# atarashansky/scrna-parameter-estimation

Hardware: NVIDIA B200
Metric: genes tested/sec (ht_1d, num_boot=10k) (higher is better)
Workload: dtype f64

## Files before the change

scrna-parameter-estimation_b200/csrc/gev.cu:

```cuda
#include "common.cuh"
#include <float.h>

namespace mm {

constexpr int kGevThreads = 64;
constexpr int kLadder = 9;
__constant__ int c_tail_n[kLadder] = {300, 270, 240, 210, 180, 150, 120, 90, 60};
__constant__ double c_ks_crit[kLadder] = {0.07783200514647708, 0.08200786390881423, 0.08693932047855427,
                                          0.09288606396320713, 0.100252942300571,   0.1097143944417969,
                                          0.12250018407843426, 0.1411693954054822,  0.1723049003305659};
constexpr double kPenalty = 709.782712893384 * 100.0;

struct GevParams {
    const double* coef_rows;
    const int* flagged;
    const int* extreme;
    int max_extreme;
    int n_flag, B, sort_cap;
    double* asl;
    int* status;
};

__device__ double gev_nnlf(const double* x, int n, double c, double loc, double scale, int lane) {
    if (!isfinite(c) || !(scale > 0.0)) return INFINITY;
    double acc = 0.0;
    int bad = 0;
    const double sup = (c > 0.0) ? 1.0 / fmax(c, DBL_MIN) : ((c < 0.0) ? 1.0 / fmin(c, -DBL_MIN) : 0.0);
    for (int i = lane; i < n; i += 32) {
        double z = (x[i] - loc) / scale;
        bool inside = (c > 0.0) ? (z < sup) : ((c < 0.0) ? (z > sup) : true);
        if (!inside || !(z == z)) { ++bad; continue; }
        double lp;
        if (c != 0.0) {
            double cx = c * z;
            double lex2 = log1p(-cx);
            double lpex2 = lex2 / c;
            lp = (cx == 1.0 || cx == -INFINITY) ? -INFINITY : (-exp(lpex2) + lpex2 - lex2);
        } else {
            lp = -exp(-z) - z;
        }
        if (isfinite(lp)) acc -= lp; else ++bad;
    }
    acc = warp_sum(acc);
    bad = warp_sum_int(bad);
    return acc + (bad > 0 ? bad * kPenalty : 0.0) + (double)n * log(scale);
}

__device__ double gev_logcdf_inner(double z, double c) {
    return (c != 0.0) ? -exp(log1p(-c * z) / c) : -exp(-z);
}
__device__ double gev_cdf(double xv, double c, double loc, double scale) {
    double z = (xv - loc) / scale;
    if (c > 0.0 && z >= 1.0 / c) return 1.0;
    if (c < 0.0 && z <= 1.0 / c) return 0.0;
    return exp(gev_logcdf_inner(z, c));
}
__device__ double gev_sf(double xv, double c, double loc, double scale) {
    double z = (xv - loc) / scale;
    if (c > 0.0 && z >= 1.0 / c) return 0.0;
    if (c < 0.0 && z <= 1.0 / c) return 1.0;
    return -expm1(gev_logcdf_inner(z, c));
}

__device__ void gev_fitstart(const double* x, int n, int lane, double th[3]) {
    double s = 0.0, mn = INFINITY, mx = -INFINITY;
    for (int i = lane; i < n; i += 32) { s += x[i]; mn = fmin(mn, x[i]); mx = fmax(mx, x[i]); }
    s = warp_sum(s);
#pragma unroll
    for (int o = 16; o > 0; o >>= 1) {
        mn = fmin(mn, __shfl_xor_sync(kFull, mn, o));
        mx = fmax(mx, __shfl_xor_sync(kFull, mx, o));
    }
    const double mu = s / n;
    double m2 = 0.0, m3 = 0.0;
    for (int i = lane; i < n; i += 32) { double d = x[i] - mu; m2 += d * d; m3 += d * d * d; }
    m2 = warp_sum(m2) / n;
    m3 = warp_sum(m3) / n;
    const double c = (m3 / pow(m2, 1.5) < 0.0) ? 0.5 : -0.5;
    double loc, scale;
    if (c > 0.0) {
        scale = sqrt(m2 / 0.8584073464102069);
        loc = mu - scale * 0.227546149094484;
        if (!isfinite(loc)) loc = 0.0;
        if (!(isfinite(scale) && scale > 0.0)) scale = 1.0;
        const double b = 2.0;
        if (!(mx < loc + b * scale)) { loc = (mx - b) + 0.1 * (mx - mn); scale = 1.0; }
    } else {
        loc = mu; scale = 1.0;
        const double a = -2.0;
        if (!(loc + a * scale < mn)) { loc = (mn - a) - 0.1 * (mx - mn); scale = 1.0; }
    }
    th[0] = c; th[1] = loc; th[2] = scale;
}

__device__ bool gev_fit(const double* x, int n, int lane, double best[3]) {
    double sim[4][3], fsim[4];
    double x0[3];
    gev_fitstart(x, n, lane, x0);
    for (int k = 0; k < 3; ++k) sim[0][k] = x0[k];
    for (int j = 0; j < 3; ++j) {
        for (int k = 0; k < 3; ++k) sim[j + 1][k] = x0[k];
        sim[j + 1][j] = (x0[j] != 0.0) ? 1.05 * x0[j] : 0.00025;
    }
    int fcalls = 0;
    for (int j = 0; j < 4; ++j) { fsim[j] = gev_nnlf(x, n, sim[j][0], sim[j][1], sim[j][2], lane); ++fcalls; }
    auto sort4 = [&]() {
        for (int i = 1; i < 4; ++i) {
            double f = fsim[i], v0 = sim[i][0], v1 = sim[i][1], v2 = sim[i][2];
            int j = i - 1;
            while (j >= 0 && fsim[j] > f) {
                fsim[j + 1] = fsim[j];
                sim[j + 1][0] = sim[j][0]; sim[j + 1][1] = sim[j][1]; sim[j + 1][2] = sim[j][2];
                --j;
            }
            fsim[j + 1] = f; sim[j + 1][0] = v0; sim[j + 1][1] = v1; sim[j + 1][2] = v2;
        }
    };
    sort4();
    const int maxit = 600, maxfun = 600;
    int it = 0;
    while (fcalls < maxfun && it < maxit) {
        double dx = 0.0, df = 0.0;
        for (int j = 1; j < 4; ++j) {
            for (int k = 0; k < 3; ++k) dx = fmax(dx, fabs(sim[j][k] - sim[0][k]));
            df = fmax(df, fabs(fsim[0] - fsim[j]));
        }
        if (dx <= 1e-4 && df <= 1e-4) break;
        double xbar[3], xr[3];
        for (int k = 0; k < 3; ++k) {
            xbar[k] = (sim[0][k] + sim[1][k] + sim[2][k]) / 3.0;
            xr[k] = 2.0 * xbar[k] - sim[3][k];
        }
        double fxr = gev_nnlf(x, n, xr[0], xr[1], xr[2], lane); ++fcalls;
        bool shrink = false;
        if (fxr < fsim[0]) {
            double xe[3];
            for (int k = 0; k < 3; ++k) xe[k] = 3.0 * xbar[k] - 2.0 * sim[3][k];
            double fxe = gev_nnlf(x, n, xe[0], xe[1], xe[2], lane); ++fcalls;
            if (fxe < fxr) { for (int k = 0; k < 3; ++k) sim[3][k] = xe[k]; fsim[3] = fxe; }
            else { for (int k = 0; k < 3; ++k) sim[3][k] = xr[k]; fsim[3] = fxr; }
        } else if (fxr < fsim[2]) {
            for (int k = 0; k < 3; ++k) sim[3][k] = xr[k];
            fsim[3] = fxr;
        } else if (fxr < fsim[3]) {
            double xc[3];
            for (int k = 0; k < 3; ++k) xc[k] = 1.5 * xbar[k] - 0.5 * sim[3][k];
            double fxc = gev_nnlf(x, n, xc[0], xc[1], xc[2], lane); ++fcalls;
            if (fxc <= fxr) { for (int k = 0; k < 3; ++k) sim[3][k] = xc[k]; fsim[3] = fxc; }
            else shrink = true;
        } else {
            double xcc[3];
            for (int k = 0; k < 3; ++k) xcc[k] = 0.5 * xbar[k] + 0.5 * sim[3][k];
            double fxcc = gev_nnlf(x, n, xcc[0], xcc[1], xcc[2], lane); ++fcalls;
            if (fxcc < fsim[3]) { for (int k = 0; k < 3; ++k) sim[3][k] = xcc[k]; fsim[3] = fxcc; }
            else shrink = true;
        }
        if (shrink) {
            for (int j = 1; j < 4; ++j) {
                for (int k = 0; k < 3; ++k) sim[j][k] = sim[0][k] + 0.5 * (sim[j][k] - sim[0][k]);
                fsim[j] = gev_nnlf(x, n, sim[j][0], sim[j][1], sim[j][2], lane); ++fcalls;
            }
        }
        sort4();
        ++it;
    }
    best[0] = sim[0][0]; best[1] = sim[0][1]; best[2] = sim[0][2];
    return isfinite(best[0]) && isfinite(best[1]) && (best[2] > 0.0);
}

__device__ double gev_ks(const double* x, int n, const double th[3], int lane) {
    double d = 0.0;
    for (int i = lane; i < n; i += 32) {
        double cdf = gev_cdf(x[i], th[0], th[1], th[2]);
        d = fmax(d, fmax((double)(i + 1) / n - cdf, cdf - (double)i / n));
    }
#pragma unroll
    for (int o = 16; o > 0; o >>= 1) d = fmax(d, __shfl_xor_sync(kFull, d, o));
    return d;
}

constexpr int kCand = 1024;

__device__ void sort_cand(double* a, int tid) {
    for (int k = 2; k <= kCand; k <<= 1)
        for (int j = k >> 1; j > 0; j >>= 1) {
            for (int i = tid; i < kCand; i += kGevThreads) {
                int l = i ^ j;
                if (l > i) {
                    double x = a[i], y = a[l];
                    bool up = ((i & k) == 0);
                    if ((x > y) == up) { a[i] = y; a[l] = x; }
                }
            }
            __syncthreads();
        }
}

__global__ void __launch_bounds__(kGevThreads)
gev_tail_kernel(GevParams P) {
    __shared__ double s_lo[kCand];
    __shared__ double s_hi[kCand];
    __shared__ double s_red[2][kGevThreads / 32];
    __shared__ int s_cnt[3];
    __shared__ int s_state[2][kLadder];
    __shared__ double s_val[2][kLadder];
    const int row = P.flagged ? P.flagged[blockIdx.x] : (int)blockIdx.x;
    if (!P.flagged) {
        const int e = P.extreme[row];
        if (e < 0 || e > P.max_extreme || !isfinite(P.asl[row])) {
            if (threadIdx.x == 0) P.status[blockIdx.x] = -1;
            return;
        }
    }
    const double* cr = P.coef_rows + (long long)row * (P.B + 1);
    const int tid = threadIdx.x, lane = tid & 31, warp = tid >> 5;
    const double stat = cr[0], astat = fabs(stat);
    if (tid < 2 * kLadder) { s_state[tid / kLadder][tid % kLadder] = 0; }
    double sum = 0.0, sq = 0.0;
    int cnt = 0;
    for (int i = tid; i < P.B; i += kGevThreads) {
        double d = cr[i + 1] - stat;
        if (isfinite(d)) { sum += d; sq = fma(d, d, sq); ++cnt; }
    }
    sum = warp_sum(sum); sq = warp_sum(sq); cnt = warp_sum_int(cnt);
    if (tid < 3) s_cnt[tid] = 0;
    if (lane == 0) { s_red[0][warp] = sum; s_red[1][warp] = sq; }
    __syncthreads();
    if (lane == 0) atomicAdd(&s_cnt[0], cnt);
    __syncthreads();
    const int n = s_cnt[0];
    double tsum = 0.0, tsq = 0.0;
    for (int w = 0; w < kGevThreads / 32; ++w) { tsum += s_red[0][w]; tsq += s_red[1][w]; }
    if (n < c_tail_n[0]) {
        if (tid == 0) P.status[blockIdx.x] = 0;
        return;
    }
    const double mu = tsum / n;
    double var = tsq / n - mu * mu;
    const double sd = sqrt(var > 0.0 ? var : 0.0);
    double t_lo = mu - 1.5 * sd, t_hi = mu + 1.5 * sd;
    bool ok_lo = false, ok_hi = false;
    for (int it = 0; it < 24 && !(ok_lo && ok_hi); ++it) {
        int c_lo = 0, c_hi = 0;
        for (int i = tid; i < P.B; i += kGevThreads) {
            double d = cr[i + 1] - stat;
            if (isfinite(d)) { c_lo += (d <= t_lo); c_hi += (d >= t_hi); }
        }
        c_lo = warp_sum_int(c_lo); c_hi = warp_sum_int(c_hi);
        __syncthreads();
        if (tid < 3) s_cnt[tid] = 0;
        __syncthreads();
        if (lane == 0) { atomicAdd(&s_cnt[1], c_lo); atomicAdd(&s_cnt[2], c_hi); }
        __syncthreads();
        c_lo = s_cnt[1]; c_hi = s_cnt[2];
        ok_lo = c_lo >= c_tail_n[0] && c_lo <= kCand;
        ok_hi = c_hi >= c_tail_n[0] && c_hi <= kCand;
        const double step = sd * (it < 8 ? 0.2 : (it < 16 ? 0.05 : 0.0125));
        if (!ok_lo) t_lo += (c_lo < c_tail_n[0]) ? step : -0.5 * step;
        if (!ok_hi) t_hi -= (c_hi < c_tail_n[0]) ? step : -0.5 * step;
    }
    if (!(ok_lo && ok_hi)) {
        if (tid == 0) P.status[blockIdx.x] = 0;
        return;
    }
    for (int i = tid; i < kCand; i += kGevThreads) { s_lo[i] = INFINITY; s_hi[i] = -INFINITY; }
    __syncthreads();
    if (tid < 3) s_cnt[tid] = 0;
    __syncthreads();
    for (int i = tid; i < P.B; i += kGevThreads) {
        double d = cr[i + 1] - stat;
        if (!isfinite(d)) continue;
        if (d <= t_lo) s_lo[atomicAdd(&s_cnt[1], 1)] = d;
        if (d >= t_hi) s_hi[atomicAdd(&s_cnt[2], 1)] = d;
    }
    __syncthreads();
    sort_cand(s_lo, tid);
    sort_cand(s_hi, tid);
    {
        const int side = warp;
        for (int li = 0; li < kLadder; ++li) {
            const int ne = c_tail_n[li];
            const double* x = side == 0 ? s_lo : s_hi + (kCand - ne);
            double th[3];
            int state;
            double val = 0.0;
            if (!gev_fit(x, ne, lane, th)) state = 3;
            else {
                double d = gev_ks(x, ne, th, lane);
                if (d < c_ks_crit[li]) {
                    state = 1;
                    double pr = side == 0 ? gev_cdf(-astat, th[0], th[1], th[2]) : gev_sf(astat, th[0], th[1], th[2]);
                    val = ((double)ne / (double)n) * pr;
                } else state = 2;
            }
            if (lane == 0) { s_state[side][li] = state; s_val[side][li] = val; }
            if (state != 2) break;
        }
    }
    __syncthreads();
    if (tid == 0) {
        double total = 0.0;
        bool ok = true;
        for (int side = 0; side < 2 && ok; ++side) {
            bool found = false;
            for (int li = 0; li < kLadder; ++li) {
                int s = s_state[side][li];
                if (s == 1) { total += s_val[side][li]; found = true; break; }
                if (s == 3 || s == 0) break;
            }
            ok = found;
        }
        if (ok && isfinite(total)) { P.asl[row] = total; P.status[blockIdx.x] = 1; }
        else P.status[blockIdx.x] = 0;
    }
}

}

using namespace mm;

MM_EXPORT int mm_gev_tail_asl(int device, void* stream, const double* coef_rows, const int32_t* flagged,
                              int32_t n_flag, int32_t num_boot, double* asl, int32_t* status,
                              const int32_t* extreme, int32_t max_extreme) {
    if (int s = enter(device)) return s;
    MM_REQUIRE(n_flag >= 0 && num_boot > 0, "n_flag/num_boot");
    if (n_flag == 0) return 0;
    MM_REQUIRE(coef_rows && (flagged || extreme) && asl && status, "null pointer");
    GevParams P;
    P.coef_rows = coef_rows; P.flagged = flagged; P.n_flag = n_flag; P.B = num_boot; P.sort_cap = 0;
    P.asl = asl; P.status = status; P.extreme = extreme; P.max_extreme = max_extreme;
    gev_tail_kernel<<<n_flag, kGevThreads, 0, (cudaStream_t)stream>>>(P);
    return check_launch("mm_gev_tail_asl");
}
```

scrna-parameter-estimation_b200/csrc/regress.cu:

```cuda
#include "common.cuh"

namespace mm {

constexpr int kRegThreads = 256;
constexpr int kMaxT = 4;
constexpr int kRegCmax = 1024;

struct FillParams {
    const double* raw_mean;
    const double* raw_rv;
    const unsigned char* seg_ok;
    const double* true_mean;
    const double* true_rv;
    const int* src_mean;
    const int* src_rv;
    const long long* gene_id;
    int R;
    int B;
    unsigned long long seed;
    double* boot_mean;
    double* boot_var;
    unsigned char* seg_good;
    int* n_valid;
    const int* n_invalid;
};

__device__ __forceinline__ double pick_valid(const double* row, int B, int n_valid, Philox& rng) {
    for (int it = 0; it < 256; ++it) {
        int j = (int)(rng.uniform() * (float)B);
        if (j >= B) j = B - 1;
        double v = row[j];
        if (v > 0.0) return v;
    }
    int want = (int)(rng.uniform() * (float)n_valid);
    if (want >= n_valid) want = n_valid - 1;
    for (int j = 0; j < B; ++j) {
        double v = row[j];
        if (v > 0.0 && want-- == 0) return v;
    }
    return nan("");
}

__global__ void __launch_bounds__(kRegThreads)
fill_log_kernel(FillParams P) {
    __shared__ int s_cnt[2];
    const long long seg = blockIdx.x;
    const int B = P.B;
    double* om = P.boot_mean + seg * (long long)(B + 1);
    double* ov = P.boot_var + seg * (long long)(B + 1);
    const double* rm = P.raw_mean + seg * (long long)B;
    const double* rr = P.raw_rv + seg * (long long)B;
    if (threadIdx.x < 2) s_cnt[threadIdx.x] = 0;
    __syncthreads();
    bool ok = P.seg_ok[seg] != 0;
    if (ok) {
        int cm = 0, cr = 0;
        for (int b = threadIdx.x; b < B; b += kRegThreads) {
            cm += (rm[b] > 0.0);
            cr += (rr[b] > 0.0);
        }
        cm = warp_sum_int(cm);
        cr = warp_sum_int(cr);
        if ((threadIdx.x & 31) == 0) { atomicAdd(&s_cnt[0], cm); atomicAdd(&s_cnt[1], cr); }
    }
    __syncthreads();
    const int nvm = s_cnt[0], nvr = s_cnt[1];
    ok = ok && nvm > 0 && nvr > 0;
    if (threadIdx.x == 0) {
        P.seg_good[seg] = ok ? 1 : 0;
        P.n_valid[2 * seg] = nvm;
        P.n_valid[2 * seg + 1] = nvr;
    }
    if (!ok) {
        for (int b = threadIdx.x; b <= B; b += kRegThreads) { om[b] = nan(""); ov[b] = nan(""); }
        return;
    }
    if (threadIdx.x == 0) { om[0] = log(P.true_mean[seg]); ov[0] = log(P.true_rv[seg]); }
    const long long sid = P.gene_id ? P.gene_id[seg / P.R] * P.R + (seg % P.R) : seg;
    for (int b = threadIdx.x; b < B; b += kRegThreads) {
        double m = rm[b], v = rr[b];
        if (!(m > 0.0)) {
            if (P.src_mean) m = rm[P.src_mean[seg * (long long)B + b]];
            else {
                Philox rng;
                rng.init(P.seed, (uint32_t)b, (uint32_t)sid, (uint32_t)(sid >> 32), 0xF111u);
                m = pick_valid(rm, B, nvm, rng);
            }
        }
        if (!(v > 0.0)) {
            if (P.src_rv) v = rr[P.src_rv[seg * (long long)B + b]];
            else {
                Philox rng;
                rng.init(P.seed, (uint32_t)b, (uint32_t)sid, (uint32_t)(sid >> 32), 0xF112u);
                v = pick_valid(rr, B, nvr, rng);
            }
        }
        om[b + 1] = log(m);
        ov[b + 1] = log(v);
    }
}

constexpr int kFillMaskWords = 2048;

__device__ __forceinline__ double pick_valid_masked(const double* row, const unsigned* mask, int B, int n_valid, Philox& rng) {
    for (int it = 0; it < 256; ++it) {
        int j = (int)(rng.uniform() * (float)B);
        if (j >= B) j = B - 1;
        if (!((mask[j >> 5] >> (j & 31)) & 1u)) return row[j];
    }
    int want = (int)(rng.uniform() * (float)n_valid);
    if (want >= n_valid) want = n_valid - 1;
    for (int j = 0; j < B; ++j)
        if (!((mask[j >> 5] >> (j & 31)) & 1u) && want-- == 0) return row[j];
    return nan("");
}

__global__ void __launch_bounds__(kRegThreads)
fill_rows_kernel(FillParams P) {
    __shared__ unsigned s_mask[2][kFillMaskWords];
    const long long seg = blockIdx.x;
    const int B = P.B;
    double* om = P.boot_mean + seg * (long long)(B + 1);
    double* ov = P.boot_var + seg * (long long)(B + 1);
    const int im = P.n_invalid[2 * seg], iv = P.n_invalid[2 * seg + 1];
    const int nvm = B - im, nvr = B - iv;
    const bool ok = P.seg_ok[seg] != 0 && nvm > 0 && nvr > 0;
    if (threadIdx.x == 0) {
        P.seg_good[seg] = ok ? 1 : 0;
        P.n_valid[2 * seg] = nvm;
        P.n_valid[2 * seg + 1] = nvr;
    }
    if (!ok) {
        for (int b = threadIdx.x; b <= B; b += kRegThreads) { om[b] = nan(""); ov[b] = nan(""); }
        return;
    }
    if (threadIdx.x == 0) { om[0] = log(P.true_mean[seg]); ov[0] = log(P.true_rv[seg]); }
    if (im == 0 && iv == 0) return;
    const int words = (B + 31) >> 5;
    for (int i = threadIdx.x; i < words; i += kRegThreads) { s_mask[0][i] = 0u; s_mask[1][i] = 0u; }
    __syncthreads();
    for (int b = threadIdx.x; b < B; b += kRegThreads) {
        if (isnan(om[b + 1])) atomicOr(&s_mask[0][b >> 5], 1u << (b & 31));
        if (isnan(ov[b + 1])) atomicOr(&s_mask[1][b >> 5], 1u << (b & 31));
    }
    __syncthreads();
    const long long sid = P.gene_id ? P.gene_id[seg / P.R] * P.R + (seg % P.R) : seg;
    for (int b = threadIdx.x; b < B; b += kRegThreads) {
        if ((s_mask[0][b >> 5] >> (b & 31)) & 1u) {
            Philox rng;
            rng.init(P.seed, (uint32_t)b, (uint32_t)sid, (uint32_t)(sid >> 32), 0xF111u);
            om[b + 1] = pick_valid_masked(om + 1, s_mask[0], B, nvm, rng);
        }
        if ((s_mask[1][b >> 5] >> (b & 31)) & 1u) {
            Philox rng;
            rng.init(P.seed, (uint32_t)b, (uint32_t)sid, (uint32_t)(sid >> 32), 0xF112u);
            ov[b + 1] = pick_valid_masked(ov + 1, s_mask[1], B, nvr, rng);
        }
    }
}

struct WlsParams {
    const double* covariate;
    const double* treatment;
    const double* weights;
    const unsigned char* masks;
    int R, Pc, T, n_mask;
    int T_full;
    const int* col_idx;
    int one_sample;
    int* one_flag;
    double* scratch;
    double* cmat;
    double* znorm2;
};

__device__ double block_sum(double v, double* sred) {
    v = warp_sum(v);
    __syncthreads();
    if ((threadIdx.x & 31) == 0) sred[threadIdx.x >> 5] = v;
    __syncthreads();
    double tot = 0.0;
    for (int w = 0; w < kRegThreads / 32; ++w) tot += sred[w];
    return tot;
}

__global__ void __launch_bounds__(kRegThreads)
wls_functional_kernel(WlsParams P) {
    __shared__ double sred[kRegThreads / 32];
    const int k = blockIdx.x;
    const int R = P.R, Pc = P.Pc, T = P.T, K = Pc + T, TF = P.T_full;
    const unsigned char* mask = P.masks + (long long)k * R;
    double* Z = P.scratch + (long long)k * R * K;
    double* C = P.cmat + (long long)k * T * R;
    const int* cols = P.col_idx ? P.col_idx + (long long)k * T : nullptr;
    const int tid = threadIdx.x;
    auto tcol = [&](int t) { return cols ? cols[t] : t; };

    double wl = 0.0, not_one = 0.0;
    for (int r = tid; r < R; r += kRegThreads) {
        if (!mask[r]) continue;
        wl += P.weights[r];
        for (int t = 0; t < T; ++t) not_one += (P.treatment[(long long)r * TF + tcol(t)] != 1.0) ? 1.0 : 0.0;
    }
    const double wsum = block_sum(wl, sred);
    const bool one_sample = P.one_sample != 0 || block_sum(not_one, sred) == 0.0;
    if (P.one_flag && tid == 0) P.one_flag[k] = one_sample ? 1 : 0;

    if (one_sample) {
        for (int i = tid; i < T * R; i += kRegThreads) {
            int r = i % R;
            C[i] = mask[r] ? P.weights[r] / wsum : 0.0;
        }
        return;
    }
    for (int c = 0; c < K; ++c) {
        double s = 0.0;
        for (int r = tid; r < R; r += kRegThreads) {
            double v = c < Pc ? P.covariate[(long long)r * Pc + c] : P.treatment[(long long)r * TF + tcol(c - Pc)];
            s += mask[r] ? P.weights[r] * v : 0.0;
        }
        double mu = block_sum(s, sred) / wsum;
        for (int r = tid; r < R; r += kRegThreads) {
            double v = c < Pc ? P.covariate[(long long)r * Pc + c] : P.treatment[(long long)r * TF + tcol(c - Pc)];
            Z[(long long)r * K + c] = mask[r] ? v - mu : 0.0;
        }
    }
    __syncthreads();
    for (int c = 0; c < Pc; ++c) {
        double s = 0.0, s0 = 0.0;
        for (int r = tid; r < R; r += kRegThreads) {
            double z = Z[(long long)r * K + c];
            s += P.weights[r] * z * z;
            double v0 = P.covariate[(long long)r * Pc + c];
            s0 += mask[r] ? P.weights[r] * v0 * v0 : 0.0;
        }
        double nrm2 = block_sum(s, sred);
        double ref2 = block_sum(s0, sred);
        const bool dropped = !(nrm2 > 1e-20 * (ref2 > 0.0 ? ref2 : 1.0));
        if (P.znorm2 && tid == 0) P.znorm2[(long long)k * Pc + c] = dropped ? 0.0 : nrm2;
        if (dropped) continue;
        for (int c2 = c + 1; c2 < K; ++c2) {
            double d = 0.0;
            for (int r = tid; r < R; r += kRegThreads)
                d += P.weights[r] * Z[(long long)r * K + c] * Z[(long long)r * K + c2];
            double proj = block_sum(d, sred) / nrm2;
            for (int r = tid; r < R; r += kRegThreads)
                Z[(long long)r * K + c2] -= proj * Z[(long long)r * K + c];
            __syncthreads();
        }
    }
    for (int t = 0; t < T; ++t) {
        double s = 0.0, s0 = 0.0;
        for (int r = tid; r < R; r += kRegThreads) {
            double a = Z[(long long)r * K + Pc + t];
            s += P.weights[r] * a * a;
            double v0 = P.treatment[(long long)r * TF + tcol(t)];
            s0 += mask[r] ? P.weights[r] * v0 * v0 : 0.0;
        }
        double ss = block_sum(s, sred);
        double ref2 = block_sum(s0, sred);
        if (!(ss > 1e-20 * (ref2 > 0.0 ? ref2 : 1.0))) ss = nan("");
        for (int r = tid; r < R; r += kRegThreads)
            C[(long long)t * R + r] = mask[r] ? P.weights[r] * Z[(long long)r * K + Pc + t] / ss : 0.0;
    }
}

struct RegParams {
    const double* boot[2];
    int n_stat;
    const unsigned char* seg_good;
    const int* mask_id;
    const int* gene_list;
    const double* cmat;
    int R, T, B;
    int approx;
    double* coef_ws;
    double* out_coef;
    double* out_se;
    double* out_asl;
    int* out_extreme;
    int* out_nnull;
    int n_split;
    double* split_ws;
};

__device__ __forceinline__ void regress_finish(const RegParams& P, long long o, double stat, double a, double b2, int h,
                                               int l, double vmin, double vmax, int n) {
    double mu = a / n, var = b2 / n - mu * mu;
    if (var < 0) var = 0;
    double sd = sqrt(var);
    double asl;
    int extreme = -1;
    if (!(vmin < vmax)) {
        asl = nan("");
    } else if (P.approx) {
        double astat = fabs(stat), k = 1.0 / (sd * 1.4142135623730951);
        asl = 0.5 * erfc((astat - mu) * k) + 0.5 * erfc((astat + mu) * k);
    } else {
        extreme = h + l;
        asl = (double)(extreme + 1) / (double)(n + 1);
    }
    P.out_coef[o] = stat;
    P.out_se[o] = (n > 0) ? sd : nan("");
    P.out_asl[o] = asl;
    P.out_extreme[o] = extreme;
    P.out_nnull[o] = n;
}

template <int TT>
__global__ void __launch_bounds__(kRegThreads)
regress_asl_kernel(RegParams P) {
    __shared__ double s_stat[2][TT];
    __shared__ double s_red[kRegThreads / 32][2 * TT][2];
    __shared__ int s_cnt[kRegThreads / 32][2 * TT][2];
    __shared__ double s_mm[kRegThreads / 32][2 * TT][2];
    __shared__ int s_nvalid[kRegThreads / 32];
    const int gi = blockIdx.x;
    const int g = P.gene_list ? P.gene_list[gi] : gi;
    const int R = P.R, T = P.T, B1 = P.B + 1, NS = P.n_stat;
    const unsigned char* good = P.seg_good + (long long)g * R;
    const double* C = P.cmat + (long long)P.mask_id[gi] * T * R;
    const int tid = threadIdx.x, lane = tid & 31, warp = tid >> 5;
    __shared__ double s_Cbuf[kRegCmax];
    __shared__ unsigned char s_good[kRegCmax];
    const double* s_C = C;
    if (T * R <= kRegCmax) {
        for (int i = tid; i < T * R; i += kRegThreads) s_Cbuf[i] = C[i];
        for (int i = tid; i < R; i += kRegThreads) s_good[i] = good[i];
        s_C = s_Cbuf;
        good = s_good;
        __syncthreads();
    }

    int n_good = 0;
    for (int r = 0; r < R; ++r) n_good += good[r];
    const long long obase = (long long)gi * NS * T;
    if (n_good == 0) {
        for (int i = tid; i < NS * T && blockIdx.y == 0; i += kRegThreads) {
            P.out_coef[obase + i] = nan(""); P.out_se[obase + i] = nan(""); P.out_asl[obase + i] = nan("");
            P.out_extreme[obase + i] = -1; P.out_nnull[obase + i] = 0;
        }
        return;
    }

    for (int t0 = 0; t0 < T; t0 += TT) {
        const int tn = min(TT, T - t0);
        if (tid < NS * tn) {
            int s = tid / tn, t = tid % tn;
            const double* bt = P.boot[s] + (long long)g * R * B1;
            double acc = 0.0;
            for (int r = 0; r < R; ++r)
                if (good[r]) acc = fma(C[(long long)(t0 + t) * R + r], bt[(long long)r * B1], acc);
            s_stat[s][t] = acc;
        }
        __syncthreads();

        double sum[2][TT], sq[2][TT], mn[2][TT], mx[2][TT];
        int hi[2][TT], lo[2][TT];
#pragma unroll
        for (int s = 0; s < 2; ++s)
#pragma unroll
            for (int t = 0; t < TT; ++t) {
                sum[s][t] = 0; sq[s][t] = 0; hi[s][t] = 0; lo[s][t] = 0;
                mn[s][t] = INFINITY; mx[s][t] = -INFINITY;
            }
        int nvalid = 0;
        const int per = (B1 + P.n_split - 1) / P.n_split;
        const int b_lo = blockIdx.y * per, b_hi = min(B1, b_lo + per);
        for (int b = b_lo + tid; b < b_hi; b += kRegThreads) {
            double acc[2][TT];
#pragma unroll
            for (int s = 0; s < 2; ++s)
#pragma unroll
                for (int t = 0; t < TT; ++t) acc[s][t] = 0.0;
            bool finite = true;
            for (int r0 = 0; r0 < R; r0 += 4) {
                double v[4][2];
#pragma unroll
                for (int j = 0; j < 4; ++j) {
                    const int r = r0 + j;
                    const bool use = r < R && good[r];
#pragma unroll
                    for (int s = 0; s < 2; ++s)
                        v[j][s] = (use && s < NS) ? __ldg(P.boot[s] + ((long long)g * R + r) * B1 + b) : 0.0;
                }
#pragma unroll
                for (int j = 0; j < 4; ++j) {
                    const int r = r0 + j;
                    if (r < R && good[r]) {
#pragma unroll
                        for (int s = 0; s < 2; ++s) {
                            finite = finite && isfinite(v[j][s]);
#pragma unroll
                            for (int t = 0; t < TT; ++t)
                                if (t < tn) acc[s][t] = fma(s_C[(t0 + t) * R + r], v[j][s], acc[s][t]);
                        }
                    }
                }
            }
#pragma unroll
            for (int s = 0; s < 2; ++s) {
                if (s < NS) {
#pragma unroll
                    for (int t = 0; t < TT; ++t) {
                        if (t < tn) {
                            double c = finite ? acc[s][t] : nan("");
                            if (P.coef_ws)
                                P.coef_ws[(((long long)gi * NS + s) * T + t0 + t) * B1 + b] = c;
                            if (finite) {
                                mn[s][t] = fmin(mn[s][t], c);
                                mx[s][t] = fmax(mx[s][t], c);
                                if (b > 0) {
                                    double st = s_stat[s][t];
                                    double d = c - st, a = fabs(st);
                                    sum[s][t] += d;
                                    sq[s][t] = fma(d, d, sq[s][t]);
                                    hi[s][t] += (d > a);
                                    lo[s][t] += (d < -a);
                                }
                            }
                        }
                    }
                }
            }
            if (finite && b > 0) ++nvalid;
        }
        nvalid = warp_sum_int(nvalid);
        if (lane == 0) s_nvalid[warp] = nvalid;
#pragma unroll
        for (int s = 0; s < 2; ++s)
#pragma unroll
            for (int t = 0; t < TT; ++t) {
                if (s < NS && t < tn) {
                    double a = warp_sum(sum[s][t]), b2 = warp_sum(sq[s][t]);
                    int h = warp_sum_int(hi[s][t]), l = warp_sum_int(lo[s][t]);
                    double vmin = mn[s][t], vmax = mx[s][t];
#pragma unroll
                    for (int o = 16; o > 0; o >>= 1) {
                        vmin = fmin(vmin, __shfl_xor_sync(kFull, vmin, o));
                        vmax = fmax(vmax, __shfl_xor_sync(kFull, vmax, o));
                    }
                    if (lane == 0) {
                        s_red[warp][s * TT + t][0] = a; s_red[warp][s * TT + t][1] = b2;
                        s_cnt[warp][s * TT + t][0] = h; s_cnt[warp][s * TT + t][1] = l;
                        s_mm[warp][s * TT + t][0] = vmin; s_mm[warp][s * TT + t][1] = vmax;
                    }
                }
            }
        __syncthreads();
        if (tid < NS * tn) {
            int s = tid / tn, t = tid % tn, j = s * TT + t;
            double a = 0, b2 = 0, vmin = INFINITY, vmax = -INFINITY;
            int h = 0, l = 0, n = 0;
            for (int w = 0; w < kRegThreads / 32; ++w) {
                a += s_red[w][j][0]; b2 += s_red[w][j][1];
                h += s_cnt[w][j][0]; l += s_cnt[w][j][1];
                vmin = fmin(vmin, s_mm[w][j][0]); vmax = fmax(vmax, s_mm[w][j][1]);
                n += s_nvalid[w];
            }
            const double stat = s_stat[s][t];
            const long long o = obase + (long long)s * T + t0 + t;
            if (P.n_split > 1) {
                double* w = P.split_ws + ((((long long)gi * P.n_split + blockIdx.y) * NS + s) * T + t0 + t) * 8;
                w[0] = a; w[1] = b2; w[2] = (double)h; w[3] = (double)l; w[4] = vmin; w[5] = vmax; w[6] = (double)n; w[7] = stat;
            } else {
                regress_finish(P, o, stat, a, b2, h, l, vmin, vmax, n);
            }
        }
        __syncthreads();
    }
}

struct ResampParams {
    double* boot[2];
    int n_stat;
    const unsigned char* seg_good;
    const int* mask_id;
    const int* gene_list;
    const double* zmat;
    const double* znorm2;
    const double* weights;
    int R, Pc, T, B;
    int approx;
    unsigned long long seed;
    const long long* gene_id;
    const int* rep_assign;
    const int* iter_assign;
    double* coef_ws;
    double* out_coef; double* out_se; double* out_asl;
    int* out_extreme; int* out_nnull;
    int* bad_flag;
};

__global__ void __launch_bounds__(kRegThreads)
regress_resampled_kernel(ResampParams P) {
    extern __shared__ int s_good[];
    __shared__ double sred[kRegThreads / 32];
    __shared__ int s_ngood;
    const int gi = blockIdx.x, tid = threadIdx.x;
    const int g = P.gene_list ? P.gene_list[gi] : gi;
    const int R = P.R, Pc = P.Pc, T = P.T, B = P.B, B1 = B + 1, K = Pc + T, NS = P.n_stat;
    const unsigned char* good = P.seg_good + (long long)g * R;
    const double* Z = P.zmat + (long long)P.mask_id[gi] * R * K;
    const double* zn = P.znorm2 + (long long)P.mask_id[gi] * Pc;
    if (tid == 0) {
        int n = 0;
        for (int r = 0; r < R; ++r) if (good[r]) s_good[n++] = r;
        s_ngood = n;
    }
    __syncthreads();
    const int ng = s_ngood;
    const long long obase = (long long)gi * NS * T;
    if (ng == 0) {
        for (int i = tid; i < NS * T; i += kRegThreads) {
            P.out_coef[obase + i] = nan(""); P.out_se[obase + i] = nan(""); P.out_asl[obase + i] = nan("");
            P.out_extreme[obase + i] = -1; P.out_nnull[obase + i] = 0;
        }
        return;
    }
    double wsum = 0.0;
    for (int i = 0; i < ng; ++i) wsum += P.weights[s_good[i]];
    for (int s = 0; s < NS; ++s) {
        double* bt = P.boot[s] + (long long)g * R * B1;
        for (int b = tid; b < B1; b += kRegThreads) {
            double mu = 0.0;
            bool finite = true;
            for (int i = 0; i < ng; ++i) {
                int r = s_good[i];
                double y = bt[(long long)r * B1 + b];
                finite = finite && isfinite(y);
                mu += P.weights[r] * y;
            }
            if (!finite) *P.bad_flag = 1;
            mu /= wsum;
            for (int i = 0; i < ng; ++i) { int r = s_good[i]; bt[(long long)r * B1 + b] -= mu; }
            for (int c = 0; c < Pc; ++c) {
                if (!(zn[c] > 0.0)) continue;
                double d = 0.0;
                for (int i = 0; i < ng; ++i) {
                    int r = s_good[i];
                    d += P.weights[r] * Z[(long long)r * K + c] * bt[(long long)r * B1 + b];
                }
                d /= zn[c];
                for (int i = 0; i < ng; ++i) { int r = s_good[i]; bt[(long long)r * B1 + b] -= d * Z[(long long)r * K + c]; }
            }
        }
    }
    __syncthreads();
    const long long sid_base = (P.gene_id ? P.gene_id[g] : (long long)g) * R;
    auto pick = [&](int i, int j, int& r, int& bi) {
        int ra;
        if (j == 0) { ra = i; bi = 0; }
        else if (P.rep_assign) {
            ra = P.rep_assign[((long long)g * R + i) * B + j];
            bi = P.iter_assign[((long long)g * R + i) * B + j];
        } else {
            Philox rng;
            long long sid = sid_base + i;
            rng.init(P.seed, (uint32_t)j, (uint32_t)sid, (uint32_t)(sid >> 32), 0x4E5Au);
            uint4 r4 = rng.block();
            ra = (int)(((unsigned long long)r4.x * (unsigned)ng) >> 32);
            bi = 1 + (int)(((unsigned long long)r4.y * (unsigned)B) >> 32);
        }
        r = s_good[ra];
    };
    auto slope = [&](const double* bt, int t, int j) {
        double sw = 0, swa = 0, swy = 0, amin = INFINITY, amax = -INFINITY;
        for (int i = 0; i < ng; ++i) {
            int r, bi;
            pick(i, j, r, bi);
            double w = P.weights[r], a = Z[(long long)r * K + Pc + t], y = bt[(long long)r * B1 + bi];
            amin = fmin(amin, a); amax = fmax(amax, a);
            sw = __dadd_rn(sw, w);
            swa = __dadd_rn(swa, __dmul_rn(a, w));
            swy = __dadd_rn(swy, __dmul_rn(y, w));
        }
        if (!(amin < amax)) return nan("");
        const double ma = swa / sw, my = swy / sw;
        double ss = 0, num = 0;
        for (int i = 0; i < ng; ++i) {
            int r, bi;
            pick(i, j, r, bi);
            double w = P.weights[r], a = Z[(long long)r * K + Pc + t], y = bt[(long long)r * B1 + bi];
            double ac = __dadd_rn(a, -ma);
            ss = __dadd_rn(ss, __dmul_rn(__dmul_rn(ac, ac), w));
            num = __dadd_rn(num, __dmul_rn(__dmul_rn(ac, w), __dadd_rn(y, -my)));
        }
        return num / sw / (ss / sw);
    };
    for (int s = 0; s < NS; ++s) {
        const double* bt = P.boot[s] + (long long)g * R * B1;
        for (int t = 0; t < T; ++t) {
            const double stat = slope(bt, t, 0);
            const double astat = fabs(stat);
            double sum = 0, sq = 0, vmin = INFINITY, vmax = -INFINITY;
            int hi = 0, lo = 0, cnt = 0;
            for (int j = tid; j < B; j += kRegThreads) {
                double c = (j == 0) ? stat : slope(bt, t, j);
                if (P.coef_ws) P.coef_ws[(((long long)gi * NS + s) * T + t) * B + j] = c;
                if (!isfinite(c)) continue;
                vmin = fmin(vmin, c); vmax = fmax(vmax, c);
                if (j > 0) {
                    double d = c - stat;
                    sum += d; sq = fma(d, d, sq); hi += (d > astat); lo += (d < -astat); ++cnt;
                }
            }
            sum = block_sum(sum, sred);
            sq = block_sum(sq, sred);
            int ext = (int)(block_sum((double)(hi + lo), sred) + 0.5);
            const int n_fin = (int)(block_sum((double)cnt, sred) + 0.5);
#pragma unroll
            for (int o = 16; o > 0; o >>= 1) {
                vmin = fmin(vmin, __shfl_xor_sync(kFull, vmin, o));
                vmax = fmax(vmax, __shfl_xor_sync(kFull, vmax, o));
            }
            __shared__ double s_mn[kRegThreads / 32], s_mx[kRegThreads / 32];
            if ((tid & 31) == 0) { s_mn[tid >> 5] = vmin; s_mx[tid >> 5] = vmax; }
            __syncthreads();
            if (tid == 0) {
                for (int w = 1; w < kRegThreads / 32; ++w) { vmin = fmin(vmin, s_mn[w]); vmax = fmax(vmax, s_mx[w]); }
                const int n = n_fin;
                double mu = sum / n, var = sq / n - mu * mu;
                if (var < 0) var = 0;
                double sd = sqrt(var), asl;
                int extreme = -1;
                if (!(vmin < vmax)) asl = nan("");
                else if (P.approx) {
                    double k2 = 1.0 / (sd * 1.4142135623730951);
                    asl = 0.5 * erfc((astat - mu) * k2) + 0.5 * erfc((astat + mu) * k2);
                } else { extreme = ext; asl = (double)(ext + 1) / (double)(n + 1); }
                const long long o = obase + (long long)s * T + t;
                P.out_coef[o] = stat; P.out_se[o] = sd; P.out_asl[o] = asl;
                P.out_extreme[o] = extreme; P.out_nnull[o] = n;
            }
            __syncthreads();
        }
    }
}

constexpr int kRsCov = 24;

__device__ __forceinline__ int build_good_list(const unsigned char* good, int R, int* s_good, int* s_n) {
    if (threadIdx.x < 32) {
        const int lane = threadIdx.x;
        int base = 0;
        for (int r0 = 0; r0 < R; r0 += 32) {
            const int r = r0 + lane;
            const bool ok = r < R && good[r];
            const unsigned m = __ballot_sync(kFull, ok);
            if (ok) s_good[base + __popc(m & ((1u << lane) - 1u))] = r;
            base += __popc(m);
        }
        if (lane == 0) *s_n = base;
    }
    __syncthreads();
    return *s_n;
}

constexpr int kRsRows = 32;
constexpr int kRsBatch = 8;

__global__ void __launch_bounds__(kRegThreads, 2)
resample_residualise_kernel(ResampParams P) {
    extern __shared__ int s_good[];
    __shared__ double sred[kRegThreads / 32];
    __shared__ int s_ngood;
    __shared__ __align__(16) double s_z[kRsRows][kRsCov];
    __shared__ double s_w[kRsRows];
    __shared__ int s_r[kRsRows];
    const int gi = blockIdx.x, tid = threadIdx.x;
    const int g = P.gene_list ? P.gene_list[gi] : gi;
    const int R = P.R, Pc = P.Pc, B1 = P.B + 1, K = Pc + P.T;
    const int ng = build_good_list(P.seg_good + (long long)g * R, R, s_good, &s_ngood);
    if (ng == 0) return;
    const double* __restrict__ Z = P.zmat + (long long)P.mask_id[gi] * R * K;
    const double* __restrict__ zn = P.znorm2 + (long long)P.mask_id[gi] * Pc;
    const double* __restrict__ wts = P.weights;
    double wl = 0.0;
    for (int i = tid; i < ng; i += kRegThreads) wl += wts[s_good[i]];
    const double wsum = block_sum(wl, sred);
    const int b = blockIdx.y * kRegThreads + tid;
    const bool active = b < B1;
    auto stage = [&](int i0, int c0, int nc, bool weighted) {
        __syncthreads();
        for (int idx = tid; idx < kRsRows * kRsCov; idx += kRegThreads) {
            const int row = idx / kRsCov, k = idx % kRsCov, i = i0 + row;
            double v = 0.0;
            if (i < ng && k < nc) {
                const int r = s_good[i];
                v = Z[(long long)r * K + c0 + k];
                if (weighted) v *= wts[r];
            }
            s_z[row][k] = v;
        }
        if (tid < kRsRows) {
            const int i = i0 + tid;
            s_r[tid] = s_good[i < ng ? i : ng - 1];
            s_w[tid] = i < ng ? wts[s_r[tid]] : 0.0;
        }
        __syncthreads();
    };
    for (int s = 0; s < P.n_stat; ++s) {
        double* __restrict__ col = P.boot[s] + (long long)g * R * B1 + (active ? b : 0);
        for (int c0 = 0; c0 == 0 || c0 < Pc; c0 += kRsCov) {
            const int nc = min(kRsCov, Pc - c0);
            double acc[kRsCov], mu = 0.0;
#pragma unroll
            for (int k = 0; k < kRsCov; ++k) acc[k] = 0.0;
            bool finite = true;
            for (int i0 = 0; i0 < ng; i0 += kRsRows) {
                stage(i0, c0, nc, true);
                if (!active) continue;
#pragma unroll 1
                for (int u0 = 0; u0 < kRsRows; u0 += kRsBatch) {
                    double y[kRsBatch];
#pragma unroll
                    for (int u = 0; u < kRsBatch; ++u) y[u] = col[(long long)s_r[u0 + u] * B1];
#pragma unroll
                    for (int u = 0; u < kRsBatch; ++u) {
                        finite = finite && (isfinite(y[u]) || s_w[u0 + u] == 0.0);
                        const double yy = s_w[u0 + u] == 0.0 ? 0.0 : y[u];
                        mu = fma(s_w[u0 + u], yy, mu);
                        const double2* zr = reinterpret_cast<const double2*>(s_z[u0 + u]);
#pragma unroll
                        for (int k = 0; k < kRsCov / 2; ++k) {
                            const double2 z2 = zr[k];
                            acc[2 * k] = fma(z2.x, yy, acc[2 * k]);
                            acc[2 * k + 1] = fma(z2.y, yy, acc[2 * k + 1]);
// ... 348 lines not shown
```

Baseline: 44280.

## Widen GEV tail fits to multi-warp sides and unroll regression over columns

The GEV tail kernel grows from one warp per tail side to four warps per side. Each side uses its own named barrier and double-buffered shared term arrays, so the per-point log-likelihood and KS work is spread over 128 threads, and both candidate arrays are sorted in a single bitonic pass. The regression kernel handles two bootstrap columns per thread for TT==1 and widens the row group to 8, which adds independent loads in flight. The cost is more barriers for each Nelder-Mead function evaluation, more shared memory and more registers.

```diff
diff --git a/scrna-parameter-estimation_b200/csrc/gev.cu b/scrna-parameter-estimation_b200/csrc/gev.cu
--- a/scrna-parameter-estimation_b200/csrc/gev.cu
+++ b/scrna-parameter-estimation_b200/csrc/gev.cu
@@ -3,13 +3,18 @@
 
 namespace mm {
 
-constexpr int kGevThreads = 64;
+constexpr int kSideWarps = 4;
+constexpr int kSideThreads = 32 * kSideWarps;
+constexpr int kGevThreads = 2 * kSideThreads;
+constexpr int kMomThreads = 64;
 constexpr int kLadder = 9;
 __constant__ int c_tail_n[kLadder] = {300, 270, 240, 210, 180, 150, 120, 90, 60};
 __constant__ double c_ks_crit[kLadder] = {0.07783200514647708, 0.08200786390881423, 0.08693932047855427,
                                           0.09288606396320713, 0.100252942300571,   0.1097143944417969,
                                           0.12250018407843426, 0.1411693954054822,  0.1723049003305659};
 constexpr double kPenalty = 709.782712893384 * 100.0;
+constexpr int kTailMax = 300;
+constexpr int kPts = (kTailMax + kSideThreads - 1) / kSideThreads;
 
 struct GevParams {
     const double* coef_rows;
@@ -21,24 +26,48 @@
     int* status;
 };
 
-__device__ double gev_nnlf(const double* x, int n, double c, double loc, double scale, int lane) {
+__device__ __forceinline__ void side_sync(int side) {
+    if (side == 0) asm volatile("bar.sync 1, %0;" ::"n"(kSideThreads) : "memory");
+    else asm volatile("bar.sync 2, %0;" ::"n"(kSideThreads) : "memory");
+}
+
+struct SideCtx {
+    int side, st, lane;
+    double* buf;
+    int phase;
+};
+
+__device__ double gev_nnlf(const double* x, int n, double c, double loc, double scale, SideCtx& S) {
     if (!isfinite(c) || !(scale > 0.0)) return INFINITY;
-    double acc = 0.0;
-    int bad = 0;
+    double* lpv = S.buf + S.phase * kTailMax;
+    S.phase ^= 1;
     const double sup = (c > 0.0) ? 1.0 / fmax(c, DBL_MIN) : ((c < 0.0) ? 1.0 / fmin(c, -DBL_MIN) : 0.0);
-    for (int i = lane; i < n; i += 32) {
-        double z = (x[i] - loc) / scale;
-        bool inside = (c > 0.0) ? (z < sup) : ((c < 0.0) ? (z > sup) : true);
-        if (!inside || !(z == z)) { ++bad; continue; }
-        double lp;
-        if (c != 0.0) {
+    if (c != 0.0) {
+#pragma unroll
+        for (int k = 0; k < kPts; ++k) {
+            const int i = S.st + k * kSideThreads;
+            double z = (x[min(i, n - 1)] - loc) / scale;
+            bool inside = (c > 0.0) ? (z < sup) : (z > sup);
             double cx = c * z;
             double lex2 = log1p(-cx);
             double lpex2 = lex2 / c;
-            lp = (cx == 1.0 || cx == -INFINITY) ? -INFINITY : (-exp(lpex2) + lpex2 - lex2);
-        } else {
-            lp = -exp(-z) - z;
-        }
+            double lp = (cx == 1.0 || cx == -INFINITY) ? -INFINITY : (-exp(lpex2) + lpex2 - lex2);
+            if (i < n) lpv[i] = (inside && z == z) ? lp : nan("");
+        }
+    } else {
+#pragma unroll
+        for (int k = 0; k < kPts; ++k) {
+            const int i = S.st + k * kSideThreads;
+            double z = (x[min(i, n - 1)] - loc) / scale;
+            double lp = -exp(-z) - z;
+            if (i < n) lpv[i] = (z == z) ? lp : nan("");
+        }
+    }
+    side_sync(S.side);
+    double acc = 0.0;
+    int bad = 0;
+    for (int i = S.lane; i < n; i += 32) {
+        double lp = lpv[i];
         if (isfinite(lp)) acc -= lp; else ++bad;
     }
     acc = warp_sum(acc);
@@ -93,17 +122,17 @@
     th[0] = c; th[1] = loc; th[2] = scale;
 }
 
-__device__ bool gev_fit(const double* x, int n, int lane, double best[3]) {
+__device__ bool gev_fit(const double* x, int n, SideCtx& S, double best[3]) {
     double sim[4][3], fsim[4];
     double x0[3];
-    gev_fitstart(x, n, lane, x0);
+    gev_fitstart(x, n, S.lane, x0);
     for (int k = 0; k < 3; ++k) sim[0][k] = x0[k];
     for (int j = 0; j < 3; ++j) {
         for (int k = 0; k < 3; ++k) sim[j + 1][k] = x0[k];
         sim[j + 1][j] = (x0[j] != 0.0) ? 1.05 * x0[j] : 0.00025;
     }
     int fcalls = 0;
-    for (int j = 0; j < 4; ++j) { fsim[j] = gev_nnlf(x, n, sim[j][0], sim[j][1], sim[j][2], lane); ++fcalls; }
+    for (int j = 0; j < 4; ++j) { fsim[j] = gev_nnlf(x, n, sim[j][0], sim[j][1], sim[j][2], S); ++fcalls; }
     auto sort4 = [&]() {
         for (int i = 1; i < 4; ++i) {
             double f = fsim[i], v0 = sim[i][0], v1 = sim[i][1], v2 = sim[i][2];
@@ -131,12 +160,12 @@
             xbar[k] = (sim[0][k] + sim[1][k] + sim[2][k]) / 3.0;
             xr[k] = 2.0 * xbar[k] - sim[3][k];
         }
-        double fxr = gev_nnlf(x, n, xr[0], xr[1], xr[2], lane); ++fcalls;
+        double fxr = gev_nnlf(x, n, xr[0], xr[1], xr[2], S); ++fcalls;
         bool shrink = false;
         if (fxr < fsim[0]) {
             double xe[3];
             for (int k = 0; k < 3; ++k) xe[k] = 3.0 * xbar[k] - 2.0 * sim[3][k];
-            double fxe = gev_nnlf(x, n, xe[0], xe[1], xe[2], lane); ++fcalls;
+            double fxe = gev_nnlf(x, n, xe[0], xe[1], xe[2], S); ++fcalls;
             if (fxe < fxr) { for (int k = 0; k < 3; ++k) sim[3][k] = xe[k]; fsim[3] = fxe; }
             else { for (int k = 0; k < 3; ++k) sim[3][k] = xr[k]; fsim[3] = fxr; }
         } else if (fxr < fsim[2]) {
@@ -145,20 +174,20 @@
         } else if (fxr < fsim[3]) {
             double xc[3];
             for (int k = 0; k < 3; ++k) xc[k] = 1.5 * xbar[k] - 0.5 * sim[3][k];
-            double fxc = gev_nnlf(x, n, xc[0], xc[1], xc[2], lane); ++fcalls;
+            double fxc = gev_nnlf(x, n, xc[0], xc[1], xc[2], S); ++fcalls;
             if (fxc <= fxr) { for (int k = 0; k < 3; ++k) sim[3][k] = xc[k]; fsim[3] = fxc; }
             else shrink = true;
         } else {
             double xcc[3];
             for (int k = 0; k < 3; ++k) xcc[k] = 0.5 * xbar[k] + 0.5 * sim[3][k];
-            double fxcc = gev_nnlf(x, n, xcc[0], xcc[1], xcc[2], lane); ++fcalls;
+            double fxcc = gev_nnlf(x, n, xcc[0], xcc[1], xcc[2], S); ++fcalls;
             if (fxcc < fsim[3]) { for (int k = 0; k < 3; ++k) sim[3][k] = xcc[k]; fsim[3] = fxcc; }
             else shrink = true;
         }
         if (shrink) {
             for (int j = 1; j < 4; ++j) {
                 for (int k = 0; k < 3; ++k) sim[j][k] = sim[0][k] + 0.5 * (sim[j][k] - sim[0][k]);
-                fsim[j] = gev_nnlf(x, n, sim[j][0], sim[j][1], sim[j][2], lane); ++fcalls;
+                fsim[j] = gev_nnlf(x, n, sim[j][0], sim[j][1], sim[j][2], S); ++fcalls;
             }
         }
         sort4();
@@ -168,14 +197,18 @@
     return isfinite(best[0]) && isfinite(best[1]) && (best[2] > 0.0);
 }
 
-__device__ double gev_ks(const double* x, int n, const double th[3], int lane) {
+__device__ double gev_ks(const double* x, int n, const double th[3], SideCtx& S, double* red) {
     double d = 0.0;
-    for (int i = lane; i < n; i += 32) {
+    for (int i = S.st; i < n; i += kSideThreads) {
         double cdf = gev_cdf(x[i], th[0], th[1], th[2]);
         d = fmax(d, fmax((double)(i + 1) / n - cdf, cdf - (double)i / n));
     }
 #pragma unroll
     for (int o = 16; o > 0; o >>= 1) d = fmax(d, __shfl_xor_sync(kFull, d, o));
+    if (S.lane == 0) red[S.st >> 5] = d;
+    side_sync(S.side);
+    for (int w = 0; w < kSideWarps; ++w) d = fmax(d, red[w]);
+    side_sync(S.side);
     return d;
 }
 
@@ -184,22 +217,23 @@
 __device__ void sort_cand(double* a, int tid) {
     for (int k = 2; k <= kCand; k <<= 1)
         for (int j = k >> 1; j > 0; j >>= 1) {
-            for (int i = tid; i < kCand; i += kGevThreads) {
-                int l = i ^ j;
+            for (int e = tid; e < 2 * kCand; e += kGevThreads) {
+                const int i = e & (kCand - 1), l = i ^ j;
                 if (l > i) {
-                    double x = a[i], y = a[l];
+                    double* b = a + (e & kCand);
+                    double x = b[i], y = b[l];
                     bool up = ((i & k) == 0);
-                    if ((x > y) == up) { a[i] = y; a[l] = x; }
+                    if ((x > y) == up) { b[i] = y; b[l] = x; }
                 }
             }
             __syncthreads();
         }
 }
 
-__global__ void __launch_bounds__(kGevThreads)
+__global__ void __launch_bounds__(kGevThreads, 2)
 gev_tail_kernel(GevParams P) {
-    __shared__ double s_lo[kCand];
-    __shared__ double s_hi[kCand];
+    __shared__ double s_cand[2][kCand];
+    __shared__ double s_terms[2][2][kTailMax];
     __shared__ double s_red[2][kGevThreads / 32];
     __shared__ int s_cnt[3];
     __shared__ int s_state[2][kLadder];
@@ -216,21 +250,23 @@
     const int tid = threadIdx.x, lane = tid & 31, warp = tid >> 5;
     const double stat = cr[0], astat = fabs(stat);
     if (tid < 2 * kLadder) { s_state[tid / kLadder][tid % kLadder] = 0; }
+    if (tid < 3) s_cnt[tid] = 0;
     double sum = 0.0, sq = 0.0;
     int cnt = 0;
-    for (int i = tid; i < P.B; i += kGevThreads) {
-        double d = cr[i + 1] - stat;
-        if (isfinite(d)) { sum += d; sq = fma(d, d, sq); ++cnt; }
-    }
-    sum = warp_sum(sum); sq = warp_sum(sq); cnt = warp_sum_int(cnt);
-    if (tid < 3) s_cnt[tid] = 0;
-    if (lane == 0) { s_red[0][warp] = sum; s_red[1][warp] = sq; }
-    __syncthreads();
-    if (lane == 0) atomicAdd(&s_cnt[0], cnt);
+    if (tid < kMomThreads) {
+        for (int i = tid; i < P.B; i += kMomThreads) {
+            double d = cr[i + 1] - stat;
+            if (isfinite(d)) { sum += d; sq = fma(d, d, sq); ++cnt; }
+        }
+        sum = warp_sum(sum); sq = warp_sum(sq); cnt = warp_sum_int(cnt);
+        if (lane == 0) { s_red[0][warp] = sum; s_red[1][warp] = sq; }
+    }
+    __syncthreads();
+    if (tid < kMomThreads && lane == 0) atomicAdd(&s_cnt[0], cnt);
     __syncthreads();
     const int n = s_cnt[0];
     double tsum = 0.0, tsq = 0.0;
-    for (int w = 0; w < kGevThreads / 32; ++w) { tsum += s_red[0][w]; tsq += s_red[1][w]; }
+    for (int w = 0; w < kMomThreads / 32; ++w) { tsum += s_red[0][w]; tsq += s_red[1][w]; }
     if (n < c_tail_n[0]) {
         if (tid == 0) P.status[blockIdx.x] = 0;
         return;
@@ -263,37 +299,38 @@
         if (tid == 0) P.status[blockIdx.x] = 0;
         return;
     }
-    for (int i = tid; i < kCand; i += kGevThreads) { s_lo[i] = INFINITY; s_hi[i] = -INFINITY; }
+    for (int i = tid; i < kCand; i += kGevThreads) { s_cand[0][i] = INFINITY; s_cand[1][i] = -INFINITY; }
     __syncthreads();
     if (tid < 3) s_cnt[tid] = 0;
     __syncthreads();
     for (int i = tid; i < P.B; i += kGevThreads) {
         double d = cr[i + 1] - stat;
         if (!isfinite(d)) continue;
-        if (d <= t_lo) s_lo[atomicAdd(&s_cnt[1], 1)] = d;
-        if (d >= t_hi) s_hi[atomicAdd(&s_cnt[2], 1)] = d;
-    }
-    __syncthreads();
-    sort_cand(s_lo, tid);
-    sort_cand(s_hi, tid);
+        if (d <= t_lo) s_cand[0][atomicAdd(&s_cnt[1], 1)] = d;
+        if (d >= t_hi) s_cand[1][atomicAdd(&s_cnt[2], 1)] = d;
+    }
+    __syncthreads();
+    sort_cand(&s_cand[0][0], tid);
     {
-        const int side = warp;
+        SideCtx S;
+        S.side = tid / kSideThreads; S.st = tid % kSideThreads; S.lane = lane;
+        S.buf = &s_terms[S.side][0][0]; S.phase = 0;
         for (int li = 0; li < kLadder; ++li) {
             const int ne = c_tail_n[li];
-            const double* x = side == 0 ? s_lo : s_hi + (kCand - ne);
+            const double* x = S.side == 0 ? s_cand[0] : s_cand[1] + (kCand - ne);
             double th[3];
             int state;
             double val = 0.0;
-            if (!gev_fit(x, ne, lane, th)) state = 3;
+            if (!gev_fit(x, ne, S, th)) state = 3;
             else {
-                double d = gev_ks(x, ne, th, lane);
+                double d = gev_ks(x, ne, th, S, &s_red[S.side][0]);
                 if (d < c_ks_crit[li]) {
                     state = 1;
-                    double pr = side == 0 ? gev_cdf(-astat, th[0], th[1], th[2]) : gev_sf(astat, th[0], th[1], th[2]);
+                    double pr = S.side == 0 ? gev_cdf(-astat, th[0], th[1], th[2]) : gev_sf(astat, th[0], th[1], th[2]);
                     val = ((double)ne / (double)n) * pr;
                 } else state = 2;
             }
-            if (lane == 0) { s_state[side][li] = state; s_val[side][li] = val; }
+            if (S.st == 0) { s_state[S.side][li] = state; s_val[S.side][li] = val; }
             if (state != 2) break;
         }
     }
diff --git a/scrna-parameter-estimation_b200/csrc/regress.cu b/scrna-parameter-estimation_b200/csrc/regress.cu
--- a/scrna-parameter-estimation_b200/csrc/regress.cu
+++ b/scrna-parameter-estimation_b200/csrc/regress.cu
@@ -310,6 +310,7 @@
 template <int TT>
 __global__ void __launch_bounds__(kRegThreads)
 regress_asl_kernel(RegParams P) {
+    constexpr int kCols = TT == 1 ? 2 : 1, kGroups = TT == 4 ? 4 : 8;
     __shared__ double s_stat[2][TT];
     __shared__ double s_red[kRegThreads / 32][2 * TT][2];
     __shared__ int s_cnt[kRegThreads / 32][2 * TT][2];
@@ -367,63 +368,78 @@
         int nvalid = 0;
         const int per = (B1 + P.n_split - 1) / P.n_split;
         const int b_lo = blockIdx.y * per, b_hi = min(B1, b_lo + per);
-        for (int b = b_lo + tid; b < b_hi; b += kRegThreads) {
-            double acc[2][TT];
-#pragma unroll
-            for (int s = 0; s < 2; ++s)
-#pragma unroll
-                for (int t = 0; t < TT; ++t) acc[s][t] = 0.0;
-            bool finite = true;
-            for (int r0 = 0; r0 < R; r0 += 4) {
-                double v[4][2];
-#pragma unroll
-                for (int j = 0; j < 4; ++j) {
+        for (int b0 = b_lo + tid; b0 < b_hi; b0 += kCols * kRegThreads) {
+            double acc[kCols][2][TT];
+            bool finite[kCols];
+#pragma unroll
+            for (int c = 0; c < kCols; ++c) {
+                finite[c] = true;
+#pragma unroll
+                for (int s = 0; s < 2; ++s)
+#pragma unroll
+                    for (int t = 0; t < TT; ++t) acc[c][s][t] = 0.0;
+            }
+            for (int r0 = 0; r0 < R; r0 += kGroups) {
+                double v[kGroups][kCols][2];
+#pragma unroll
+                for (int j = 0; j < kGroups; ++j) {
                     const int r = r0 + j;
                     const bool use = r < R && good[r];
 #pragma unroll
-                    for (int s = 0; s < 2; ++s)
-                        v[j][s] = (use && s < NS) ? __ldg(P.boot[s] + ((long long)g * R + r) * B1 + b) : 0.0;
-                }
-#pragma unroll
-                for (int j = 0; j < 4; ++j) {
+                    for (int s = 0; s < 2; ++s) {
+                        const double* row = P.boot[s] + ((long long)g * R + r) * B1 + b0;
+#pragma unroll
+                        for (int c = 0; c < kCols; ++c)
+                            v[j][c][s] = (use && s < NS && b0 + c * kRegThreads < b_hi) ? __ldg(row + c * kRegThreads) : 0.0;
+                    }
+                }
+#pragma unroll
+                for (int j = 0; j < kGroups; ++j) {
                     const int r = r0 + j;
                     if (r < R && good[r]) {
 #pragma unroll
-                        for (int s = 0; s < 2; ++s) {
-                            finite = finite && isfinite(v[j][s]);
-#pragma unroll
-                            for (int t = 0; t < TT; ++t)
-                                if (t < tn) acc[s][t] = fma(s_C[(t0 + t) * R + r], v[j][s], acc[s][t]);
-                        }
+                        for (int c = 0; c < kCols; ++c)
+#pragma unroll
+                            for (int s = 0; s < 2; ++s) {
+                                finite[c] = finite[c] && isfinite(v[j][c][s]);
+#pragma unroll
+                                for (int t = 0; t < TT; ++t)
+                                    if (t < tn) acc[c][s][t] = fma(s_C[(t0 + t) * R + r], v[j][c][s], acc[c][s][t]);
+                            }
                     }
                 }
             }
 #pragma unroll
-            for (int s = 0; s < 2; ++s) {
-                if (s < NS) {
-#pragma unroll
-                    for (int t = 0; t < TT; ++t) {
-                        if (t < tn) {
-                            double c = finite ? acc[s][t] : nan("");
-                            if (P.coef_ws)
-                                P.coef_ws[(((long long)gi * NS + s) * T + t0 + t) * B1 + b] = c;
-                            if (finite) {
-                                mn[s][t] = fmin(mn[s][t], c);
-                                mx[s][t] = fmax(mx[s][t], c);
-                                if (b > 0) {
-                                    double st = s_stat[s][t];
-                                    double d = c - st, a = fabs(st);
-                                    sum[s][t] += d;
-                                    sq[s][t] = fma(d, d, sq[s][t]);
-                                    hi[s][t] += (d > a);
-                                    lo[s][t] += (d < -a);
+            for (int c = 0; c < kCols; ++c) {
+                const int b = b0 + c * kRegThreads;
+                if (b >= b_hi) break;
+#pragma unroll
+                for (int s = 0; s < 2; ++s) {
+                    if (s < NS) {
+#pragma unroll
+                        for (int t = 0; t < TT; ++t) {
+                            if (t < tn) {
+                                double cf = finite[c] ? acc[c][s][t] : nan("");
+                                if (P.coef_ws)
+                                    P.coef_ws[(((long long)gi * NS + s) * T + t0 + t) * B1 + b] = cf;
+                                if (finite[c]) {
+                                    mn[s][t] = fmin(mn[s][t], cf);
+                                    mx[s][t] = fmax(mx[s][t], cf);
+                                    if (b > 0) {
+                                        double st = s_stat[s][t];
+                                        double d = cf - st, a = fabs(st);
+                                        sum[s][t] += d;
+                                        sq[s][t] = fma(d, d, sq[s][t]);
+                                        hi[s][t] += (d > a);
+                                        lo[s][t] += (d < -a);
+                                    }
                                 }
                             }
                         }
                     }
                 }
-            }
-            if (finite && b > 0) ++nvalid;
+                if (finite[c] && b > 0) ++nvalid;
+            }
         }
         nvalid = warp_sum_int(nvalid);
         if (lane == 0) s_nvalid[warp] = nvalid;
```

New measurement: 44520 (median of 6 runs). About the same (+0.5%).
